# petuum/poseidon

Measured on AMD Instinct MI355X. Metric: images/sec (whole node), higher is better.
Workload: dtype bf16; 1 GPU; model=alexnet, global_batch=256, input=3x227x227, parallelism=dp1, sfb=False, hipgraph=True

## Files before the change

### poseidon_amd/ops/csrc/bindings.cpp

```cpp

#include <torch/extension.h>
#include <c10/hip/HIPStream.h>
#include <hip/hip_runtime.h>

#include <algorithm>
#include <atomic>
#include <cmath>
#include <cstdlib>
#include <utility>

#include "ps_api.h"
#include "ps_mt.h"

namespace {

using at::Tensor;

hipStream_t stream() { return c10::hip::getCurrentHIPStream().stream(); }

bool is_bf16(const Tensor& t) { return t.scalar_type() == at::kBFloat16; }

struct P {
  void* p;
  explicit P(const Tensor& t) : p(t.data_ptr()) {}
// ... 33 lines not shown
  return t_cl.permute({0, 2, 3, 1}).reshape({NP, t_cl.size(1)});
}

Tensor as_rows(const Tensor& t, int64_t* rows, int* C) {
  Tensor tc = t.dim() == 4 ? cl4(t) : t.contiguous();
  *C = (int)(t.dim() == 4 ? tc.size(1) : tc.size(-1));
  *rows = tc.numel() / *C;
  return tc;
}

Tensor weight_shadow(const Tensor& w_f32, bool bf16) {
  if (!bf16) return w_f32.contiguous();
  auto wc = w_f32.contiguous();
  Tensor out = at::empty(wc.sizes(), wc.options().dtype(at::kBFloat16));
  ps_f32_to_bf16(wc.data_ptr<float>(), out.data_ptr(), wc.numel(), stream());
  return out;
}


std::atomic<bool> g_implicit_gemm{false};
std::atomic<int64_t> g_implicit_thresh{192LL << 20};
std::atomic<int64_t> g_dgrad_fwd_thresh{128LL << 20};
std::atomic<bool> g_packed_conv{false};

void set_implicit_gemm(bool on) { g_implicit_gemm.store(on); }
void set_packed_conv(bool on) { g_packed_conv.store(on); }
void set_implicit_threshold(int64_t bytes) { g_implicit_thresh.store(bytes); }
void set_dgrad_fwd_threshold(int64_t bytes) { g_dgrad_fwd_thresh.store(bytes); }

bool deterministic() { return ps_deterministic() != 0; }
void set_deterministic(bool on) { ps_set_deterministic(on ? 1 : 0); }
int64_t float_atomic_launches(bool reset) {
  return ps_float_atomic_launches(reset ? 1 : 0);
}

void colsum_into(const Tensor& d, float* out, int64_t R, int C) {
  Tensor scratch;
  const int64_t n = ps_colsum_scratch_elems(R, C, is_bf16(d) ? 1 : 0);
  if (n > 0) scratch = at::empty({n}, d.options().dtype(at::kFloat));
  PS_CALL(colsum, is_bf16(d), P(d), out, R, C,
          n > 0 ? scratch.data_ptr<float>() : nullptr, stream());
}

const void* zero_page(const Tensor& like) {
  static Tensor z;
  if (!z.defined())
    z = at::zeros({64}, like.options().dtype(at::kByte));
// ... 139 lines not shown
    if (own) dw = t;
  }
  if (has_bias) {
    Tensor t = at::zeros({N}, x.options().dtype(at::kFloat));
    colsum_into(dyc, t.data_ptr<float>(), M, N);
    db = t;
  }
  return {dx, dw, db};
}

Tensor gemm_at_b(const Tensor& a, const Tensor& b) {
  check_float_like(a, "a");
  auto ac = a.contiguous();
  auto bc = b.contiguous();
  int M = ac.size(0), N = ac.size(1), K = bc.size(1);
  Tensor t = at::empty({N, K}, a.options().dtype(at::kFloat));
  run_gemm(ac, bc, t, nullptr, N, K, M, N, K, K, 0, 0, 0, false, false,
           1.0f, 0.0f);
  return t;
}


enum { PS_PACKED_OFF = 0, PS_PACKED_ON = 1, PS_PACKED_AUTO = -1 };

ConvPlan conv_plan_for(at::IntArrayRef x_shape, int Co, int kh, int kw,
                       int sh, int sw, int ph, int pw, int G, bool bf16,
                       int packed = PS_PACKED_AUTO) {
  TORCH_CHECK(x_shape.size() == 4 && G > 0 && x_shape[1] % G == 0 &&
              Co % G == 0, "conv channel/group mismatch");
  const ConvPolicy policy = {
      g_implicit_gemm.load(), g_implicit_thresh.load(),
      g_dgrad_fwd_thresh.load(),
      packed == PS_PACKED_AUTO ? g_packed_conv.load() : packed == PS_PACKED_ON};
  return ps_conv_plan((int)x_shape[0], (int)x_shape[1], (int)x_shape[2],
                      (int)x_shape[3], Co, kh, kw, sh, sw, ph, pw, G,
                      bf16 ? 2 : 4, policy);
}

py::dict conv_plan(std::vector<int64_t> x_shape, std::vector<int64_t> w_shape,
                   std::vector<int64_t> stride, std::vector<int64_t> pad,
                   int G, bool bf16) {
  TORCH_CHECK(w_shape.size() == 4 && stride.size() == 2 && pad.size() == 2);
  TORCH_CHECK(x_shape.size() == 4 && w_shape[1] * G == x_shape[1],
              "conv channel/group mismatch");
  const ConvPlan p = conv_plan_for(x_shape, (int)w_shape[0], (int)w_shape[2],
                                   (int)w_shape[3], (int)stride[0],
                                   (int)stride[1], (int)pad[0], (int)pad[1],
                                   G, bf16);
  py::dict d;
  d["N"] = p.g.N; d["C"] = p.g.C; d["H"] = p.g.H; d["W"] = p.g.W;
  d["Ho"] = p.g.Ho; d["Wo"] = p.g.Wo; d["G"] = p.g.G;
  d["Co"] = p.Co; d["Cg"] = p.Cg; d["Cog"] = p.Cog;
  d["Kg"] = p.Kg; d["Kcol"] = p.Kcol; d["NP"] = p.NP; d["vec"] = p.vec;
  d["is_1x1"] = p.is_1x1; d["ld_col"] = p.ld_col; d["wk_ld"] = p.wk_ld;
  d["kpad"] = p.kpad; d["implicit"] = p.implicit;
  d["Kgw_implicit"] = p.Kgw_implicit; d["dgrad_as_fwd"] = p.dgrad_as_fwd;
  d["packed"] = p.packed; d["pk_W"] = p.pk_W; d["pk_kw"] = p.pk_kw;
  d["pk_Kg"] = p.pk_Kg; d["kw_ld"] = p.kw_ld; d["c_ld"] = p.c_ld;
  d["Kgw"] = p.implicit ? p.Kgw_implicit : p.wk_ld;
  return d;
}

std::vector<int64_t> khwc_layout(int64_t Cg, int64_t kw, bool packed) {
  int kw_ld, c_ld;
  ps_khwc_layout((int)kw, (int)Cg, packed, &kw_ld, &c_ld);
  return {kw_ld, c_ld};
}

Tensor weight_khwc_tr(const Tensor& w, int G, bool bf16) {
  auto wc = w.contiguous();
  int Co = wc.size(0), Cig = wc.size(1), kh = wc.size(2), kw = wc.size(3);
  int Kg = kh * kw * Cig;
  Tensor wkT = at::empty({(int64_t)G * Kg, (int64_t)(Co / G)},
                         w.options().dtype(bf16 ? at::kBFloat16 : at::kFloat));
  PS_CALL_W(weight_to_khwc_tr, bf16, wc.data_ptr<float>(), P(wkT), Co, Cig,
          kh, kw, G, stream());
  return wkT;
}

std::vector<Tensor> conv2d_forward_ex(const Tensor& x, const Tensor& w,
                                      const c10::optional<Tensor>& bias,
// ... 11 lines not shown
  const ConvGeom& g = p.g;
  const int Co = p.Co, Cog = p.Cog;
  Tensor x_cl = (p.is_1x1 || p.implicit) ? cl4(x) : Tensor();

  const auto cdt = bf16 ? at::kBFloat16 : at::kFloat;
  Tensor wk, wkT;
  if (wk_cached.has_value() && wkT_cached.has_value() &&
      wk_cached->scalar_type() == cdt) {
    TORCH_CHECK(wk_cached->size(1) == p.wk_ld, "conv2d_forward: cached wk is ",
                wk_cached->size(1), " wide, the plan's wk_ld is ", p.wk_ld);
    wk = *wk_cached;
    wkT = *wkT_cached;
  } else {
    auto wc = w.contiguous();
    auto wkopts = w.options().dtype(cdt);
    wk = p.kpad ? at::zeros({Co, (int64_t)p.wk_ld}, wkopts)
                : at::empty({Co, (int64_t)p.wk_ld}, wkopts);
    wkT = at::empty({(int64_t)p.Kcol, (int64_t)Cog}, wkopts);
    PS_CALL_W(weight_to_khwc_both, bf16, wc.data_ptr<float>(), P(wk), P(wkT),
            Co, p.Cg, g.kh, g.kw, G, p.wk_ld, p.kw_ld, p.c_ld, stream());
  }

  Tensor colT;
  if (p.packed) {
    colT = at::empty({g.N, g.H, (int64_t)p.pk_W, PS_PK_C}, x.options());
    ps_pack_pairs_bf16(x.data_ptr(), colT.data_ptr(), g.N, g.C, g.H, g.W,
                       p.pk_W, g.pw, x.stride(0), x.stride(1), x.stride(2),
                       x.stride(3), stream());
  } else if (p.is_1x1) {
    colT = rows2d(x_cl);
  } else if (!p.implicit) {
    colT = at::empty({p.NP, (int64_t)p.ld_col}, x.options());
    const bool staged = PS_CALL(im2col_rowstage, bf16, P(x), P(colT), &g,
                                p.ld_col, x.stride(0), x.stride(1),
                                x.stride(2), x.stride(3), stream());
    if (!staged) {
      const Tensor xc = cl4(x);
      PS_CALL(im2col_nhwc, bf16, P(xc), P(colT), &g, p.ld_col, stream());
      if (p.kpad)
        PS_CALL(zero_cols, bf16, P(colT), p.NP, p.ld_col, p.Kcol, stream());
    }
  }

  Tensor y = empty_cl({g.N, Co, g.Ho, g.Wo}, x.options());
  const float* bp = nullptr;
  Tensor bc;
// ... 69 lines not shown
  for (int grp = 0; grp < G; ++grp) {
    run_gemm(dy2, wkT, dcolT, nullptr,
             (int)p.NP, Kg, Cog,
             Co, Cog, p.Kcol,
             (int64_t)grp * Cog, (int64_t)grp * Kg * Cog,
             (int64_t)grp * Kg,
             true, true, 1.0f, 0.0f);
  }
  if (!p.is_1x1)
    PS_CALL(col2im_nhwc, bf16, P(dcolT), P(dx), &g, stream());
  return dx;
}

Tensor conv2d_backward_weight_acc(const Tensor& x, const Tensor& colT,
                                  const Tensor& dy, Tensor dw_out,
                                  c10::optional<Tensor> db_out,
                                  int sh, int sw, int ph, int pw, int G,
                                  const c10::optional<Tensor>& dwk_buf,
                                  bool skip_unpack, bool skip_db) {
  check_float_like(dy, "dy");
  auto dy_cl = cl4(dy);
  const bool implicit = colT.numel() == 0 && colT.dim() == 1;
  const bool packed = colT.dim() == 4;
  const ConvPlan p = conv_plan_for(x.sizes(), (int)dw_out.size(0),
                                   (int)dw_out.size(2), (int)dw_out.size(3),
                                   sh, sw, ph, pw, G, is_bf16(dy),
                                   packed ? PS_PACKED_ON : PS_PACKED_OFF);
  TORCH_CHECK(dw_out.size(1) == p.Cg && dy_cl.size(2) == p.g.Ho &&
              dy_cl.size(3) == p.g.Wo, "conv wgrad: shape mismatch");
  const int Co = p.Co, Cog = p.Cog;
  if (packed) {
    TORCH_CHECK(p.packed && colT.is_contiguous() && is_bf16(colT) &&
                colT.size(0) == p.g.N && colT.size(1) == p.g.H &&
                colT.size(2) == p.pk_W && colT.size(3) == PS_PK_C,
                "conv wgrad: packed input does not match the plan");
  } else {
    TORCH_CHECK(implicit || colT.size(1) == p.ld_col,
                "conv wgrad: colT width does not match the plan");
  }
  const Tensor xg = packed ? colT : implicit ? cl4(x) : Tensor();
  const bool gather = implicit || packed;
  const int Kgw = implicit ? p.Kgw_implicit : p.wk_ld;

  const bool prez = dwk_buf.has_value() && dwk_buf->numel() == (int64_t)Co * Kgw;
  Tensor dwk = prez ? *dwk_buf
             : at::empty({Co, (int64_t)Kgw}, dy.options().dtype(at::kFloat));
  Tensor dy2 = rows2d(dy_cl);
  for (int grp = 0; grp < G; ++grp) {
    GatherDesc gb{};
    if (gather)
      gb = ps_gather_desc(p, PS_GATHER_WGRAD, xg.data_ptr(), zero_page(xg),
                          grp);
    run_gemm(dy2, gather ? xg : colT, dwk, nullptr,
// ... 872 lines not shown
}

PYBIND11_MODULE(TORCH_EXTENSION_NAME, m) {
  m.def("data_transform", &data_transform);
  m.def("gemm", &gemm);
  m.def("gemm_plan", &gemm_plan);
  m.def("linear_forward", &linear_forward);
  m.def("linear_backward", &linear_backward);
  m.def("gemm_at_b", &gemm_at_b);
  m.def("conv_plan", &conv_plan);
  m.def("conv2d_forward_ex", &conv2d_forward_ex);
  m.def("conv2d_backward_input", &conv2d_backward_input);
  m.def("conv2d_backward_weight_acc", &conv2d_backward_weight_acc);
  m.def("set_implicit_gemm", &set_implicit_gemm);
  m.def("set_deterministic", &set_deterministic);
  m.def("deterministic", &deterministic);
  m.def("float_atomic_launches", &float_atomic_launches);
  m.def("set_tr16_tune", &ps_gemm_set_tr_tune);
  m.def("set_implicit_threshold", &set_implicit_threshold);
  m.def("set_packed_conv", &set_packed_conv);
  m.def("khwc_layout", &khwc_layout);
  if (const char* e = std::getenv("PS_PACKED_CONV"))
    set_packed_conv(std::atoi(e) != 0);
  m.def("set_dgrad_fwd_threshold", &set_dgrad_fwd_threshold);
  m.def("concat_channels", &concat_channels);
  m.def("slice_channels", &slice_channels);
  m.def("split_channels", &split_channels);
  m.def("pool_max_forward", &pool_max_forward);
  m.def("pool_max_backward", &pool_max_backward);
  m.def("pool_ave_forward", &pool_ave_forward);
  m.def("pool_ave_backward", &pool_ave_backward);
  m.def("pool_stoch_forward_train", &pool_stoch_forward_train);
  m.def("pool_stoch_forward_test", &pool_stoch_forward_test);
  m.def("lrn_forward", &lrn_forward);
  m.def("lrn_backward", &lrn_backward);
  m.def("lrn_backward_tail", &lrn_backward_tail);
  m.def("pool_max_backward_tail", &pool_max_backward_tail);
  m.def("relu_backward_bias", &relu_backward_bias);
  m.def("set_bwd_tail_blocks", &set_bwd_tail_blocks);
  m.def("lrn_v8_ok", &ps_lrn_v8_ok);
  m.def("softmax_forward", &softmax_forward);
  m.def("softmax_backward", &softmax_backward);
  m.def("softmax_loss_forward", &softmax_loss_forward);
  m.def("softmax_loss_backward", &softmax_loss_backward);
  m.def("relu_forward", &relu_forward);
  m.def("relu_backward", &relu_backward);
// ... 31 lines not shown
```

### poseidon_amd/ops/csrc/ps_api.h

```cpp
#pragma once
#include <hip/hip_runtime.h>
#include <cstdint>

#include "ps_conv_plan.h"
#include "ps_gemm_plan.h"
#include "ps_transform.h"

struct GemmArgs {
  const void* A;
  const void* B;
  void* C;
  const float* bias;
  int M, N, K;
  int64_t lda, ldb, ldc;
  float alpha, beta;
  bool a_klast, b_klast;
  bool in_bf16;
  bool out_f32;
  const GatherDesc* gather_a;
  const GatherDesc* gather_b;
  bool relu;
  bool c_prezeroed;
};

// ... 126 lines not shown
                   hipStream_t);
void ps_nesterov_update(float*, const float*, float*, int64_t, float, float,
                        float, hipStream_t);
void ps_adagrad_update(float*, const float*, float*, int64_t, float, float,
                       float, hipStream_t);
void ps_f32_to_bf16(const float*, void*, int64_t, hipStream_t);
void ps_sgd_update_lrdev(float*, const float*, float*, int64_t, float, float,
                         float, const float*, hipStream_t);
void ps_u64_inc(void*, hipStream_t);
void ps_sgd_mt(const void* descs, const void* chunks, int nchunks, float lr,
               float mom, const float* lr_dev, hipStream_t);
void ps_zero_mt(const void* descs, const void* chunks, int nchunks,
                hipStream_t);
void ps_repack_mt(const void* descs, const void* chunks, int nchunks,
                  hipStream_t);
void ps_unpack_mt(const void* descs, const void* chunks, int nchunks,
                  hipStream_t);

void ps_data_transform_f32(const uint8_t*, const int*, const float*, float*,
                           const TransformGeom*, hipStream_t);
void ps_data_transform_bf16(const uint8_t*, const int*, const float*, void*,
                            const TransformGeom*, hipStream_t);

void ps_chan_concat4_f32(float*, void* const*, const int*, int, int, int64_t,
                         int, int, const void* const*, hipStream_t);
void ps_chan_concat4_bf16(void*, void* const*, const int*, int, int, int64_t,
                          int, int, const void* const*, hipStream_t);
void ps_chan_copy_f32(const float*, float*, int64_t, int, int, int, hipStream_t);
void ps_chan_copy_bf16(const void*, void*, int64_t, int, int, int, hipStream_t);
void ps_chan_slice_f32(const float*, float*, int64_t, int, int, int, hipStream_t);
void ps_chan_slice_bf16(const void*, void*, int64_t, int, int, int, hipStream_t);
void ps_im2col_nhwc_f32(const float*, float*, const ConvGeom*, int ldcol,
                        hipStream_t);
bool ps_im2col_rowstage_f32(const float*, float*, const ConvGeom*, int ldcol,
                            int64_t sn, int64_t sc, int64_t sh, int64_t sw,
                            hipStream_t);
bool ps_im2col_rowstage_bf16(const void*, void*, const ConvGeom*, int ldcol,
                             int64_t sn, int64_t sc, int64_t sh, int64_t sw,
                             hipStream_t);
void ps_col2im_nhwc_f32(const float*, float*, const ConvGeom*, hipStream_t);
void ps_im2col_nhwc_bf16(const void*, void*, const ConvGeom*, int ldcol,
                         hipStream_t);
void ps_col2im_nhwc_bf16(const void*, void*, const ConvGeom*, hipStream_t);
void ps_weight_to_khwc_f32(const float*, float*, int, int, int, int, hipStream_t);
void ps_weight_to_khwc_f32_bf16(const float*, void*, int, int, int, int, hipStream_t);
void ps_zero_cols_f32(float*, int64_t rows, int ld, int c_lo, hipStream_t);
// ... 23 lines not shown
```

### poseidon_amd/ops/csrc/ps_conv_plan.h

```cpp
#pragma once
#include <cstdint>

#if defined(__HIPCC__)
#define PS_HD __host__ __device__
#else
#define PS_HD
#endif

struct ConvGeom {
  int N, C, H, W;
  int Ho, Wo;
  int kh, kw, sh, sw, ph, pw;
  int G;
};

struct GatherDesc {
  const void* x;
  const void* zero;
  int C, H, W, Ho, Wo;
  int kh, kw, sh, sw, ph, pw;
  int Cg, c0;
  int kg_max;
  float inv_Cg, inv_kw, inv_Wo, inv_Ho;
};

inline void ps_fill_gather_inv(GatherDesc* g) {
  g->inv_Cg = 1.0f / g->Cg;
  g->inv_kw = 1.0f / g->kw;
  g->inv_Wo = 1.0f / g->Wo;
  g->inv_Ho = 1.0f / g->Ho;
}

struct ConvPolicy {
  bool force_implicit;
  int64_t implicit_bytes;
  int64_t dgrad_fwd_bytes;
  bool packed;
};

constexpr int PS_PK_SLOTS = 4;
constexpr int PS_PK_C = 2 * PS_PK_SLOTS;

PS_HD inline int ps_pk_chunk(int iw, int pw) { return (iw + pw) >> 1; }
PS_HD inline int ps_pk_half(int iw, int pw) { return (iw + pw) & 1; }
PS_HD inline int64_t ps_pk_x_index(int n, int ih, int iw, int c, int H,
                                   int Wp, int pw) {
  return (((int64_t)n * H + ih) * Wp + ps_pk_chunk(iw, pw)) * PS_PK_C +
         ps_pk_half(iw, pw) * PS_PK_SLOTS + c;
}
PS_HD inline int ps_khwc_col(int ky, int kx, int c, int kw_ld, int c_ld) {
  return (ky * kw_ld + kx) * c_ld + c;
}
inline void ps_khwc_layout(int kw, int Cg, bool packed, int* kw_ld,
                           int* c_ld) {
  *kw_ld = packed ? 2 * ((kw + 1) / 2) : kw;
  *c_ld = packed ? PS_PK_SLOTS : Cg;
}

struct ConvPlan {
  ConvGeom g;
  int Co, Cg, Cog;
  int Kg, Kcol;
  int64_t NP;
  int vec;
  bool is_1x1;
  int ld_col;
  int wk_ld;
  bool kpad;
  bool implicit;
  int Kgw_implicit;
  bool dgrad_as_fwd;
  bool packed;
  int pk_W;
  int pk_kw;
  int pk_Kg;
  int kw_ld, c_ld;
};

inline ConvPlan ps_conv_plan(int N, int C, int H, int W, int Co, int kh,
                             int kw, int sh, int sw, int ph, int pw, int G,
                             int elem_bytes, const ConvPolicy& policy) {
  ConvPlan p;
  p.g = {N, C, H, W, (H + 2 * ph - kh) / sh + 1, (W + 2 * pw - kw) / sw + 1,
         kh, kw, sh, sw, ph, pw, G};
  p.Co = Co;
  p.Cg = C / G;
  p.Cog = Co / G;
  p.Kg = kh * kw * p.Cg;
  p.Kcol = G * p.Kg;
  p.NP = (int64_t)N * p.g.Ho * p.g.Wo;
  p.vec = 16 / elem_bytes;
  p.is_1x1 = kh == 1 && kw == 1 && sh == 1 && sw == 1 && ph == 0 && pw == 0;
  p.ld_col = (p.is_1x1 || G != 1) ? p.Kcol : (p.Kcol + 63) & ~63;
  p.wk_ld = p.ld_col / G;
  p.kpad = p.ld_col != p.Kcol;
  const int64_t colT_bytes = p.NP * p.Kcol * elem_bytes;
  p.implicit = (policy.force_implicit || colT_bytes > policy.implicit_bytes) &&
               !p.is_1x1 && p.Cg % p.vec == 0;
  p.Kgw_implicit = (p.Kg + 63) & ~63;
  p.packed = policy.packed && G == 1 &&
             C <= PS_PK_SLOTS && elem_bytes == 2 && sw % 2 == 0 && !p.is_1x1 &&
             p.g.Ho > 0 && p.g.Wo > 0;
  p.pk_kw = (kw + 1) / 2;
  p.pk_W = (p.g.Wo - 1) * (sw / 2) + p.pk_kw;
  p.pk_Kg = kh * p.pk_kw * PS_PK_C;
  ps_khwc_layout(kw, p.Cg, p.packed, &p.kw_ld, &p.c_ld);
  if (p.packed) {
    p.implicit = false;
    p.wk_ld = (p.pk_Kg + 63) & ~63;
    p.kpad = true;
  }
  p.dgrad_as_fwd = sh == 1 && sw == 1 && !p.is_1x1 && p.Cog % p.vec == 0 &&
                   ph <= kh - 1 && pw <= kw - 1 &&
                   colT_bytes > policy.dgrad_fwd_bytes;
  return p;
}

enum ConvGatherRole {
  PS_GATHER_FWD,
  PS_GATHER_WGRAD,
  PS_GATHER_DGRAD_AS_FWD,
};

inline GatherDesc ps_gather_desc(const ConvPlan& p, ConvGatherRole role,
                                 const void* x, const void* zero, int grp) {
  const ConvGeom& g = p.g;
  GatherDesc d;
  d.x = x;
  d.zero = zero;
  d.kh = g.kh; d.kw = g.kw;
  if (role == PS_GATHER_DGRAD_AS_FWD) {
    d.C = p.Co; d.H = g.Ho; d.W = g.Wo; d.Ho = g.H; d.Wo = g.W;
    d.sh = 1; d.sw = 1; d.ph = g.kh - 1 - g.ph; d.pw = g.kw - 1 - g.pw;
    d.Cg = p.Cog; d.c0 = grp * p.Cog;
// ... 17 lines not shown
```

### poseidon_amd/ops/functional.py

```python

from __future__ import annotations

import math
import os
from typing import Optional, Tuple

import torch
import torch.nn.functional as F

_EXT = None
_EXT_ERR: Optional[str] = None


def _ext():
    global _EXT, _EXT_ERR
    if _EXT is None and _EXT_ERR is None:
        try:
            from . import _backend
            _EXT = _backend.load()
        except Exception as e:
            _EXT_ERR = str(e)
    if _EXT is None:
        raise RuntimeError(
            "poseidon_amd HIP extension is not built/loadable but a GPU op was "
            f"requested. Build it with `python setup.py build_ext --inplace` "
            f"(PYTORCH_ROCM_ARCH=gfx950). Original error: {_EXT_ERR}")
    return _EXT


def set_implicit_gemm(on: bool) -> None:
    _ext().set_implicit_gemm(bool(on))


def set_implicit_threshold(bytes_: int) -> None:
    if ext_available():
        _ext().set_implicit_threshold(int(bytes_))


_conv_policy_epoch = 0


def set_packed_conv(on: bool) -> None:
    global _conv_policy_epoch
    _ext().set_packed_conv(bool(on))
    _conv_policy_epoch += 1


def conv_policy_epoch() -> int:
    return _conv_policy_epoch


_deterministic_cpu = os.environ.get("PS_DETERMINISTIC", "0") not in ("", "0")


def set_deterministic(on: bool) -> None:
    global _deterministic_cpu, _conv_policy_epoch
    on = bool(on)
    if on == deterministic():
        return
    if ext_available():
        _ext().set_deterministic(on)
    _deterministic_cpu = on
    _conv_policy_epoch += 1
    from ..core.context import ctx
    ctx().deterministic = on


def deterministic() -> bool:
# ... 655 lines not shown
```

### setup.py

```python

import os

os.environ.setdefault("PYTORCH_ROCM_ARCH", "gfx950")

from setuptools import setup
from torch.utils.cpp_extension import BuildExtension, CUDAExtension

CSRC = os.path.join("poseidon_amd", "ops", "csrc")

sources = [
    os.path.join(CSRC, f)
    for f in [
        "bindings.cpp",
        "gemm.hip",
        "elementwise.hip",
        "pool.hip",
        "lrn.hip",
        "softmax.hip",
        "sgd.hip",
        "im2col.hip",
        "transform.hip",
    ]
]

_cxx = ["-O3"]
_ld = []
if os.environ.get("PS_SANITIZE") == "address":
    _cxx += ["-fsanitize=address", "-fno-omit-frame-pointer", "-g"]
    _ld += ["-fsanitize=address"]
elif os.environ.get("PS_SANITIZE") == "thread":
    _cxx += ["-fsanitize=thread", "-fno-omit-frame-pointer", "-g"]
    _ld += ["-fsanitize=thread"]

setup(
    name="poseidon_amd_hip",
    ext_modules=[
        CUDAExtension(
            name="poseidon_amd.ops._hip",
            sources=sources,
            extra_compile_args={
                "cxx": _cxx,
                "nvcc": ["-O3", "-std=c++17"],
            },
# ... 6 lines not shown
```

Measured before the change: 61030 images/sec.

## Add row-fused implicit bf16 conv for small-channel layers, skipping im2col

Adds a row-fused convolution path for forward and weight-gradient passes. It is used for bf16, ungrouped, non-1x1 convs whose channel count is not vector-aligned and whose im2col buffer would be large, which fits the AlexNet first layer. Instead of materialising a large im2col column matrix, each block stages a strip of input rows in LDS, double-buffered by dedicated stager waves. It gathers the GEMM operands from LDS through a k-offset table and runs MFMA directly, fusing bias and ReLU in forward. The wgrad path accumulates with float atomics, so it is not deterministic and is turned off when determinism is requested. The in-LDS gathers may limit MFMA throughput.

Measured after the change: 62240 images/sec (median of 6 runs). +2.0%, better.

```diff
diff --git a/poseidon_amd/ops/csrc/bindings.cpp b/poseidon_amd/ops/csrc/bindings.cpp
--- a/poseidon_amd/ops/csrc/bindings.cpp
+++ b/poseidon_amd/ops/csrc/bindings.cpp
@@ -79,7 +79,13 @@
 std::atomic<int64_t> g_implicit_thresh{192LL << 20};
 std::atomic<int64_t> g_dgrad_fwd_thresh{128LL << 20};
 std::atomic<bool> g_packed_conv{false};
-
+std::atomic<bool> g_rowfused_conv{true};
+std::atomic<int64_t> g_rowfused_thresh{256LL << 20};
+
+void set_rowfused_conv(bool on) { g_rowfused_conv.store(on); }
+bool rowfused_conv() { return g_rowfused_conv.load(); }
+int64_t rowfused_threshold() { return g_rowfused_thresh.load(); }
+void set_rowfused_threshold(int64_t bytes) { g_rowfused_thresh.store(bytes); }
 void set_implicit_gemm(bool on) { g_implicit_gemm.store(on); }
 void set_packed_conv(bool on) { g_packed_conv.store(on); }
 void set_implicit_threshold(int64_t bytes) { g_implicit_thresh.store(bytes); }
@@ -265,19 +271,27 @@
 
 
 enum { PS_PACKED_OFF = 0, PS_PACKED_ON = 1, PS_PACKED_AUTO = -1 };
+enum { PS_ROWFUSED_OFF = 0, PS_ROWFUSED_ON = 1, PS_ROWFUSED_AUTO = -1 };
 
 ConvPlan conv_plan_for(at::IntArrayRef x_shape, int Co, int kh, int kw,
                        int sh, int sw, int ph, int pw, int G, bool bf16,
-                       int packed = PS_PACKED_AUTO) {
+                       int packed = PS_PACKED_AUTO,
+                       int rowfused = PS_ROWFUSED_AUTO) {
   TORCH_CHECK(x_shape.size() == 4 && G > 0 && x_shape[1] % G == 0 &&
               Co % G == 0, "conv channel/group mismatch");
+  const bool rf_auto = rowfused == PS_ROWFUSED_AUTO;
   const ConvPolicy policy = {
       g_implicit_gemm.load(), g_implicit_thresh.load(),
       g_dgrad_fwd_thresh.load(),
-      packed == PS_PACKED_AUTO ? g_packed_conv.load() : packed == PS_PACKED_ON};
-  return ps_conv_plan((int)x_shape[0], (int)x_shape[1], (int)x_shape[2],
-                      (int)x_shape[3], Co, kh, kw, sh, sw, ph, pw, G,
-                      bf16 ? 2 : 4, policy);
+      packed == PS_PACKED_AUTO ? g_packed_conv.load() : packed == PS_PACKED_ON,
+      rf_auto ? g_rowfused_conv.load() : rowfused == PS_ROWFUSED_ON,
+      rf_auto ? g_rowfused_thresh.load() : 0,
+      rf_auto && ps_deterministic() != 0};
+  ConvPlan p = ps_conv_plan((int)x_shape[0], (int)x_shape[1], (int)x_shape[2],
+                            (int)x_shape[3], Co, kh, kw, sh, sw, ph, pw, G,
+                            bf16 ? 2 : 4, policy);
+  if (p.rowfused && !ps_rowfused_prepare()) p.rowfused = false;
+  return p;
 }
 
 py::dict conv_plan(std::vector<int64_t> x_shape, std::vector<int64_t> w_shape,
@@ -300,6 +314,7 @@
   d["Kgw_implicit"] = p.Kgw_implicit; d["dgrad_as_fwd"] = p.dgrad_as_fwd;
   d["packed"] = p.packed; d["pk_W"] = p.pk_W; d["pk_kw"] = p.pk_kw;
   d["pk_Kg"] = p.pk_Kg; d["kw_ld"] = p.kw_ld; d["c_ld"] = p.c_ld;
+  d["rowfused"] = p.rowfused;
   d["Kgw"] = p.implicit ? p.Kgw_implicit : p.wk_ld;
   return d;
 }
@@ -357,6 +372,27 @@
   }
 
   Tensor colT;
+  if (p.rowfused) {
+    TORCH_CHECK(x.numel() / g.N < (1LL << 31) &&
+                (g.H - 1) * x.stride(2) + (g.W - 1) * x.stride(3) +
+                (g.C - 1) * x.stride(1) < (1LL << 31),
+                "row-fused conv: one image must span < 2^31 elements");
+    TORCH_CHECK(wk.is_contiguous() && ((uintptr_t)wk.data_ptr() & 15) == 0,
+                "row-fused conv: wk must be contiguous and 16 B aligned");
+    const RowFusedTiling t = ps_rowfused_tiling(
+        g.N, g.C, g.H, g.W, Co, g.kh, g.kw, g.sh, g.sw, g.ph, g.pw, p.wk_ld);
+    Tensor y = empty_cl({g.N, Co, g.Ho, g.Wo}, x.options());
+    Tensor bc;
+    const float* bp = nullptr;
+    if (bias.has_value()) {
+      bc = bias->contiguous();
+      bp = bc.data_ptr<float>();
+    }
+    ps_conv_rowfused_fwd(&t, x.data_ptr(), x.stride(0), x.stride(1),
+                         x.stride(2), x.stride(3), wk.data_ptr(), bp,
+                         y.data_ptr(), fuse_relu ? 1 : 0, stream());
+    return {y, at::empty({0, (int64_t)p.ld_col}, x.options()), wkT};
+  }
   if (p.packed) {
     colT = at::empty({g.N, g.H, (int64_t)p.pk_W, PS_PK_C}, x.options());
     ps_pack_pairs_bf16(x.data_ptr(), colT.data_ptr(), g.N, g.C, g.H, g.W,
@@ -472,13 +508,43 @@
   auto dy_cl = cl4(dy);
   const bool implicit = colT.numel() == 0 && colT.dim() == 1;
   const bool packed = colT.dim() == 4;
+  const bool rowfused = colT.dim() == 2 && colT.size(0) == 0;
   const ConvPlan p = conv_plan_for(x.sizes(), (int)dw_out.size(0),
                                    (int)dw_out.size(2), (int)dw_out.size(3),
                                    sh, sw, ph, pw, G, is_bf16(dy),
-                                   packed ? PS_PACKED_ON : PS_PACKED_OFF);
+                                   packed ? PS_PACKED_ON : PS_PACKED_OFF,
+                                   rowfused ? PS_ROWFUSED_ON : PS_ROWFUSED_OFF);
   TORCH_CHECK(dw_out.size(1) == p.Cg && dy_cl.size(2) == p.g.Ho &&
               dy_cl.size(3) == p.g.Wo, "conv wgrad: shape mismatch");
   const int Co = p.Co, Cog = p.Cog;
+  if (rowfused) {
+    TORCH_CHECK(p.rowfused && is_bf16(x) && is_bf16(dy),
+                "conv wgrad: row-fused cache slot does not match the plan");
+    TORCH_CHECK(!ps_deterministic(),
+                "conv wgrad: the row-fused wgrad has no deterministic form");
+    const ConvGeom& g = p.g;
+    TORCH_CHECK(x.numel() / g.N < (1LL << 31) &&
+                (g.H - 1) * x.stride(2) + (g.W - 1) * x.stride(3) +
+                (g.C - 1) * x.stride(1) < (1LL << 31),
+                "row-fused conv: one image must span < 2^31 elements");
+    const int Kgw = p.wk_ld;
+    const bool prez =
+        dwk_buf.has_value() && dwk_buf->numel() == (int64_t)Co * Kgw;
+    Tensor dwk = prez ? *dwk_buf
+               : at::empty({Co, (int64_t)Kgw}, dy.options().dtype(at::kFloat));
+    const RowFusedTiling t = ps_rowfused_tiling(
+        g.N, g.C, g.H, g.W, Co, g.kh, g.kw, g.sh, g.sw, g.ph, g.pw, p.wk_ld);
+    ps_conv_rowfused_wgrad(&t, x.data_ptr(), x.stride(0), x.stride(1),
+                           x.stride(2), x.stride(3), dy_cl.data_ptr(),
+                           dwk.data_ptr<float>(), prez ? 1 : 0, stream());
+    if (!skip_unpack)
+      ps_weight_from_khwc_f32(dwk.data_ptr<float>(), dw_out.data_ptr<float>(),
+                              Co, p.Cg, g.kh, g.kw, Kgw,
+                              1.0f, p.kw_ld, p.c_ld, stream());
+    if (db_out.has_value() && !skip_db)
+      colsum_into(dy_cl, db_out->data_ptr<float>(), p.NP, Co);
+    return dwk;
+  }
   if (packed) {
     TORCH_CHECK(p.packed && colT.is_contiguous() && is_bf16(colT) &&
                 colT.size(0) == p.g.N && colT.size(1) == p.g.H &&
@@ -1397,6 +1463,13 @@
   m.def("khwc_layout", &khwc_layout);
   if (const char* e = std::getenv("PS_PACKED_CONV"))
     set_packed_conv(std::atoi(e) != 0);
+  m.def("set_rowfused_conv", &set_rowfused_conv);
+  m.def("set_rowfused_threshold", &set_rowfused_threshold);
+  m.def("rowfused_conv", &rowfused_conv);
+  m.def("rowfused_threshold", &rowfused_threshold);
+  m.def("set_rowfused_blocks", &ps_rowfused_set_blocks);
+  if (const char* e = std::getenv("PS_ROWFUSED_CONV"))
+    set_rowfused_conv(std::atoi(e) != 0);
   m.def("set_dgrad_fwd_threshold", &set_dgrad_fwd_threshold);
   m.def("concat_channels", &concat_channels);
   m.def("slice_channels", &slice_channels);
diff --git a/poseidon_amd/ops/csrc/conv_rowfused.hip b/poseidon_amd/ops/csrc/conv_rowfused.hip
--- /dev/null
+++ b/poseidon_amd/ops/csrc/conv_rowfused.hip
@@ -0,0 +1,453 @@
+
+#include "ps_common.h"
+#include "ps_api.h"
+#include "ps_rowfused.h"
+
+#include <atomic>
+#include <mutex>
+
+namespace ps {
+namespace {
+
+constexpr int RF_THREADS = PS_RF_THREADS;
+constexpr int RF_STAGERS = 256;
+
+typedef __attribute__((ext_vector_type(4))) __bf16 rf_bf16x4;
+typedef __attribute__((ext_vector_type(4))) int rf_i32x4;
+
+struct RfX {
+  const __bf16* x;
+  int64_t sn;
+  int sc, sh, sw;
+};
+
+__device__ inline __bf16 rf_read(const char* img, int pbase, int koff) {
+  return *reinterpret_cast<const __bf16*>(img + max(pbase + koff, 0));
+}
+
+typedef __bf16 rf_uvec8 __attribute__((ext_vector_type(8), aligned(2)));
+
+template <int NV, int NT>
+__device__ inline void rf_load_x(bf16x8 (&xv)[NV], const RowFusedTiling& t,
+                                 const RowFusedTile& tl, const RfX& X,
+                                 int tid, int first) {
+  const int vpr = t.rsw_ld / 8;
+  const int total = t.srows * t.C * vpr;
+  const int iw0 = tl.ow0 * t.sw - t.pw;
+  const int ih0 = tl.oh0 * t.sh - t.ph;
+  const __bf16* xn = X.x + tl.n * X.sn;
+#pragma unroll
+  for (int v = 0; v < NV; ++v) {
+    const int idx = first + tid + v * NT;
+    const int rc = idx / vpr;
+    const int sr = rc / t.C;
+    const int c = rc - sr * t.C;
+    const int ih = ih0 + sr;
+    const int iw = iw0 + (idx - rc * vpr) * 8;
+#pragma unroll
+    for (int j = 0; j < 8; ++j) xv[v][j] = (__bf16)0.0f;
+    if (idx < total && ih >= 0 && ih < t.H) {
+      const __bf16* src = xn + (ih * X.sh + c * X.sc);
+      if (X.sw == 1 && iw >= 0 && iw + 8 <= t.W) {
+        xv[v] = *reinterpret_cast<const rf_uvec8*>(src + iw);
+      } else {
+#pragma unroll
+        for (int j = 0; j < 8; ++j)
+          if (iw + j >= 0 && iw + j < t.W) xv[v][j] = src[(iw + j) * X.sw];
+      }
+    }
+  }
+}
+
+template <int NV, int NT>
+__device__ inline void rf_store_x(char* img, const bf16x8 (&xv)[NV],
+                                  const RowFusedTiling& t, int tid,
+                                  int first) {
+  const int total = t.srows * t.C * (t.rsw_ld / 8);
+#pragma unroll
+  for (int v = 0; v < NV; ++v) {
+    const int idx = first + tid + v * NT;
+    if (idx < total)
+      *reinterpret_cast<bf16x8*>(img + PS_RF_HDR + idx * 16) = xv[v];
+  }
+}
+
+constexpr int RF_FV = 6;
+__device__ inline void rf_stage_x(char* img, const RowFusedTiling& t,
+                                  const RowFusedTile& tl, const RfX& X,
+                                  int ptid) {
+  const int total = t.srows * t.C * (t.rsw_ld / 8);
+  for (int first = 0; first < total; first += RF_FV * RF_STAGERS) {
+    bf16x8 xv[RF_FV];
+    rf_load_x<RF_FV, RF_STAGERS>(xv, t, tl, X, ptid, first);
+    rf_store_x<RF_FV, RF_STAGERS>(img, xv, t, ptid, first);
+  }
+}
+
+__device__ inline void rf_zero_headers(char* xs0, int xs_bytes, int tid) {
+  if (tid < 4) reinterpret_cast<int*>(xs0)[tid] = 0;
+  else if (tid < 8) reinterpret_cast<int*>(xs0 + xs_bytes)[tid - 4] = 0;
+}
+
+template <int FN>
+__global__ __launch_bounds__(RF_THREADS)
+void conv_rowfused_fwd_k(RowFusedTiling t, RfX X,
+                         const __bf16* __restrict__ wk,
+                         const float* __restrict__ bias,
+                         __bf16* __restrict__ y, int relu, float alpha,
+                         int tpb) {
+  extern __shared__ __attribute__((aligned(16))) char smem[];
+  __bf16* wl = reinterpret_cast<__bf16*>(smem);
+  int* kofft = reinterpret_cast<int*>(smem + t.fwd_koff_off);
+  char* xs0 = smem + t.fwd_xs_off;
+  const int tid = threadIdx.x;
+  const int lane = tid & 63;
+  const int wid = __builtin_amdgcn_readfirstlane(tid >> 6);
+  const int l = lane & 15, q = lane >> 4;
+  const int64_t t0 = (int64_t)blockIdx.x * tpb;
+  const int64_t t1 = t0 + tpb < t.tiles ? t0 + tpb : t.tiles;
+  if (t0 >= t1) return;
+
+  {
+    const int vpr = t.Kpad / 8;
+    for (int i = tid; i < t.Cop * vpr; i += RF_THREADS) {
+      const int co = i / vpr;
+      const int kv = (i - co * vpr) * 8;
+      bf16x8 v;
+#pragma unroll
+      for (int j = 0; j < 8; ++j) v[j] = (__bf16)0.0f;
+      if (co < t.Co)
+        v = *reinterpret_cast<const bf16x8*>(&wk[(int64_t)co * t.Kpad + kv]);
+      *reinterpret_cast<bf16x8*>(&wl[co * t.w_ld + kv]) = v;
+    }
+    for (int k = tid; k < t.Kpad; k += RF_THREADS) kofft[k] = ps_rf_koff(t, k);
+    rf_zero_headers(xs0, t.xs_bytes, tid);
+  }
+  if (wid >= 4)
+    rf_stage_x(xs0, t, ps_rf_tile(t, t0), X, tid - RF_STAGERS);
+  int pf[2], pbf[2];
+#pragma unroll
+  for (int f = 0; f < 2; ++f) {
+    pf[f] = (wid & 3) * 32 + f * 16 + l;
+    pbf[f] = ps_rf_pbase(t, pf[f]);
+  }
+  __syncthreads();
+
+  for (int64_t ti = t0; ti < t1; ++ti) {
+    const int cur = (int)(ti - t0) & 1;
+    if (wid >= 4) {
+      if (ti + 1 < t1)
+        rf_stage_x(xs0 + (cur ^ 1) * t.xs_bytes, t, ps_rf_tile(t, ti + 1), X,
+                   tid - RF_STAGERS);
+    } else {
+      const RowFusedTile tl = ps_rf_tile(t, ti);
+      if (wid * 32 < tl.nlive) {
+        const char* img = xs0 + cur * t.xs_bytes;
+        int pb[2];
+#pragma unroll
+        for (int f = 0; f < 2; ++f)
+          pb[f] = pf[f] < tl.nlive ? pbf[f] : PS_RF_NEG;
+        f32x4 acc[2][FN] = {};
+#pragma unroll 2
+        for (int ks = 0; ks < t.Kpad; ks += 32) {
+          const rf_i32x4 k0 =
+              *reinterpret_cast<const rf_i32x4*>(&kofft[ks + q * 8]);
+          const rf_i32x4 k1 =
+              *reinterpret_cast<const rf_i32x4*>(&kofft[ks + q * 8 + 4]);
+          bf16x8 bfr[FN];
+#pragma unroll
+          for (int fn = 0; fn < FN; ++fn)
+            bfr[fn] = *reinterpret_cast<const bf16x8*>(
+                &wl[(fn * 16 + l) * t.w_ld + ks + q * 8]);
+          bf16x8 af[2];
+#pragma unroll
+          for (int f = 0; f < 2; ++f) {
+#pragma unroll
+            for (int e = 0; e < 4; ++e) {
+              af[f][e] = rf_read(img, pb[f], k0[e]);
+              af[f][4 + e] = rf_read(img, pb[f], k1[e]);
+            }
+          }
+#pragma unroll
+          for (int f = 0; f < 2; ++f)
+#pragma unroll
+            for (int fn = 0; fn < FN; ++fn)
+              acc[f][fn] = __builtin_amdgcn_mfma_f32_16x16x32_bf16(
+                  af[f], bfr[fn], acc[f][fn], 0, 0, 0);
+        }
+#pragma unroll
+        for (int f = 0; f < 2; ++f) {
+#pragma unroll
+          for (int fn = 0; fn < FN; ++fn) {
+            const int col = fn * 16 + l;
+            if (col >= t.Co) continue;
+            const float bv = bias ? bias[col] : 0.0f;
+#pragma unroll
+            for (int r = 0; r < 4; ++r) {
+              const int p = wid * 32 + f * 16 + q * 4 + r;
+              if (p >= tl.nlive) continue;
+              float v = alpha * acc[f][fn][r] + bv;
+              if (relu && v < 0.0f) v = 0.0f;
+              from_f32(v, y[(tl.pos0 + p) * t.Co + col]);
+            }
+          }
+        }
+      }
+    }
+    __syncthreads();
+  }
+}
+
+__device__ inline bf16x8 rf_tr_frag(unsigned base, int kk, int cb, int l,
+                                    int ld) {
+  const unsigned a1 =
+      base + (unsigned)(((kk + (l >> 2)) * ld + cb + 4 * (l & 3)) * 2);
+  const unsigned a2 = a1 + (unsigned)(4 * ld * 2);
+  rf_bf16x4 v1, v2;
+  asm volatile("ds_read_b64_tr_b16 %0, %2\n\t"
+               "ds_read_b64_tr_b16 %1, %3"
+               : "=&v"(v1), "=&v"(v2) : "v"(a1), "v"(a2));
+  bf16x8 f;
+#pragma unroll
+  for (int i = 0; i < 4; ++i) { f[i] = v1[i]; f[4 + i] = v2[i]; }
+  return f;
+}
+
+template <int N>
+__device__ inline void rf_tr_wait(bf16x8 (&a)[N]) {
+  asm volatile("s_waitcnt lgkmcnt(0)" ::: "memory");
+#pragma unroll
+  for (int i = 0; i < N; ++i) asm volatile("" : "+v"(a[i]));
+}
+
+template <int FN, int KF>
+__global__ __launch_bounds__(RF_THREADS)
+void conv_rowfused_wgrad_k(RowFusedTiling t, RfX X,
+                           const __bf16* __restrict__ dy,
+                           float* __restrict__ dwk, int tpb) {
+  extern __shared__ __attribute__((aligned(16))) char smem[];
+  int* ptab = reinterpret_cast<int*>(smem);
+  __bf16* dyl0 = reinterpret_cast<__bf16*>(smem + t.wg_dy_off);
+  char* xs0 = smem + t.wg_xs_off;
+  const int dy_tile = PS_RF_TM * t.dy_ld;
+  const int tid = threadIdx.x;
+  const int lane = tid & 63;
+  const int wid = __builtin_amdgcn_readfirstlane(tid >> 6);
+  const int l = lane & 15, q = lane >> 4;
+  const int64_t t0 = (int64_t)blockIdx.x * tpb;
+  const int64_t t1 = t0 + tpb < t.tiles ? t0 + tpb : t.tiles;
+  if (t0 >= t1) return;
+  rf_zero_headers(xs0, t.xs_bytes, tid);
+
+  const int my_pb = tid < PS_RF_TM ? ps_rf_pbase(t, tid) : 0;
+  const int cv8 = t.Cop / 8;
+  bf16x8 xv[PS_RF_XV], dv[PS_RF_DV];
+  auto load = [&](int64_t ti) {
+    const RowFusedTile tl = ps_rf_tile(t, ti);
+    rf_load_x<PS_RF_XV, RF_THREADS>(xv, t, tl, X, tid, 0);
+#pragma unroll
+    for (int v = 0; v < PS_RF_DV; ++v) {
+      const int idx = tid + v * RF_THREADS;
+      const int p = idx / cv8;
+      const int cv = (idx - p * cv8) * 8;
+#pragma unroll
+      for (int j = 0; j < 8; ++j) dv[v][j] = (__bf16)0.0f;
+      if (p < tl.nlive && cv < t.Co)
+        dv[v] = *reinterpret_cast<const bf16x8*>(
+            &dy[(tl.pos0 + p) * t.Co + cv]);
+    }
+  };
+  auto store = [&](int buf, int64_t ti) {
+    const RowFusedTile tl = ps_rf_tile(t, ti);
+    rf_store_x<PS_RF_XV, RF_THREADS>(xs0 + buf * t.xs_bytes, xv, t, tid,
+                                     0);
+    __bf16* dyl = dyl0 + buf * dy_tile;
+#pragma unroll
+    for (int v = 0; v < PS_RF_DV; ++v) {
+      const int idx = tid + v * RF_THREADS;
+      const int p = idx / cv8;
+      const int cv = (idx - p * cv8) * 8;
+      if (p < PS_RF_TM)
+        *reinterpret_cast<bf16x8*>(&dyl[p * t.dy_ld + cv]) = dv[v];
+    }
+    if (tid < PS_RF_TM)
+      ptab[buf * PS_RF_TM + tid] = tid < tl.nlive ? my_pb : PS_RF_NEG;
+  };
+  load(t0);
+  store(0, t0);
+
+  const int by = blockIdx.y;
+  int kofs[KF];
+  bool klive[KF];
+#pragma unroll
+  for (int i = 0; i < KF; ++i) {
+    const int kf = (by * KF + i) * 8 + wid;
+    klive[i] = kf * 16 < t.Kpad;
+    kofs[i] = klive[i] ? ps_rf_koff(t, kf * 16 + l) : PS_RF_NEG;
+  }
+  f32x4 acc[FN][KF] = {};
+  __syncthreads();
+
+  for (int64_t ti = t0; ti < t1; ++ti) {
+    const int cur = (int)(ti - t0) & 1;
+    if (ti + 1 < t1) load(ti + 1);
+    {
+      const RowFusedTile tl = ps_rf_tile(t, ti);
+      const char* img = xs0 + cur * t.xs_bytes;
+      const int* pt = ptab + cur * PS_RF_TM;
+      const unsigned dyb = (unsigned)(unsigned long long)(
+          __attribute__((address_space(3))) __bf16*)(dyl0 + cur * dy_tile);
+      for (int p0 = 0; p0 < tl.nlive; p0 += 32) {
+        const rf_i32x4 pa =
+            *reinterpret_cast<const rf_i32x4*>(&pt[p0 + q * 8]);
+        const rf_i32x4 pb =
+            *reinterpret_cast<const rf_i32x4*>(&pt[p0 + q * 8 + 4]);
+        bf16x8 af[FN];
+#pragma unroll
+        for (int fn = 0; fn < FN; ++fn)
+          af[fn] = rf_tr_frag(dyb, p0 + q * 8, fn * 16, l, t.dy_ld);
+        rf_tr_wait(af);
+#pragma unroll
+        for (int i = 0; i < KF; ++i) {
+          if (klive[i]) {
+            bf16x8 bfr;
+#pragma unroll
+            for (int e = 0; e < 4; ++e) {
+              bfr[e] = rf_read(img, pa[e], kofs[i]);
+              bfr[4 + e] = rf_read(img, pb[e], kofs[i]);
+            }
+#pragma unroll
+            for (int fn = 0; fn < FN; ++fn)
+              acc[fn][i] = __builtin_amdgcn_mfma_f32_16x16x32_bf16(
+                  af[fn], bfr, acc[fn][i], 0, 0, 0);
+          }
+        }
+      }
+    }
+    if (ti + 1 < t1) store(cur ^ 1, ti + 1);
+    __syncthreads();
+  }
+#pragma unroll
+  for (int fn = 0; fn < FN; ++fn)
+#pragma unroll
+    for (int i = 0; i < KF; ++i) {
+      if (!klive[i]) continue;
+      const int k = ((by * KF + i) * 8 + wid) * 16 + l;
+      if (k >= t.Kcol) continue;
+#pragma unroll
+      for (int r = 0; r < 4; ++r) {
+        const int co = fn * 16 + q * 4 + r;
+        if (co < t.Co)
+          atomicAdd(&dwk[(int64_t)co * t.Kpad + k], acc[fn][i][r]);
+      }
+    }
+}
+
+std::atomic<int> g_rf_blocks{0};
+
+std::atomic<int> g_rf_cus{0};
+std::once_flag g_rf_once;
+
+int rf_cu_count() {
+  const int n = g_rf_cus.load();
+  return n > 0 ? n : 256;
+}
+
+void rf_grid(const RowFusedTiling& t, int* blocks, int* tpb) {
+  const int cap = g_rf_blocks.load();
+  int64_t b = cap > 0 ? cap : rf_cu_count();
+  if (b > t.tiles) b = t.tiles;
+  *tpb = (int)((t.tiles + b - 1) / b);
+  *blocks = (int)((t.tiles + *tpb - 1) / *tpb);
+}
+
+template <typename K>
+bool rf_allow_lds(K kernel) {
+  return hipFuncSetAttribute(reinterpret_cast<const void*>(kernel),
+                             hipFuncAttributeMaxDynamicSharedMemorySize,
+                             PS_RF_LDS_MAX) == hipSuccess;
+}
+
+template <int FN>
+void rf_launch_fwd(const RowFusedTiling& t, const RfX& X, const void* wk,
+                   const float* bias, void* y, int relu, hipStream_t s) {
+  int blocks, tpb;
+  rf_grid(t, &blocks, &tpb);
+  conv_rowfused_fwd_k<FN><<<dim3((unsigned)blocks), RF_THREADS, t.fwd_lds,
+                            s>>>(t, X, (const __bf16*)wk, bias, (__bf16*)y,
+                                 relu, 1.0f, tpb);
+}
+
+template <int FN, int KF>
+void rf_launch_wgrad(const RowFusedTiling& t, const RfX& X, const void* dy,
+                     float* dwk, hipStream_t s) {
+  int blocks, tpb;
+  rf_grid(t, &blocks, &tpb);
+  const int gy = (t.Kpad / 16 + 8 * KF - 1) / (8 * KF);
+  conv_rowfused_wgrad_k<FN, KF><<<dim3((unsigned)blocks, (unsigned)gy),
+                                  RF_THREADS, t.wg_lds, s>>>(
+      t, X, (const __bf16*)dy, dwk, tpb);
+}
+
+}
+}
+
+extern "C" {
+
+void ps_rowfused_set_blocks(int n) { ps::g_rf_blocks.store(n < 0 ? 0 : n); }
+
+int ps_rowfused_prepare() {
+  using namespace ps;
+  std::call_once(g_rf_once, [] {
+    int dev = 0, n = 0;
+    if (hipGetDevice(&dev) != hipSuccess ||
+        hipDeviceGetAttribute(&n, hipDeviceAttributeMultiprocessorCount,
+                              dev) != hipSuccess || n <= 0)
+      return;
+    const bool ok =
+        rf_allow_lds(conv_rowfused_fwd_k<1>) &&
+        rf_allow_lds(conv_rowfused_fwd_k<2>) &&
+        rf_allow_lds(conv_rowfused_fwd_k<4>) &&
+        rf_allow_lds(conv_rowfused_fwd_k<6>) &&
+        rf_allow_lds(conv_rowfused_fwd_k<8>) &&
+        rf_allow_lds(conv_rowfused_wgrad_k<1, 3>) &&
+        rf_allow_lds(conv_rowfused_wgrad_k<2, 3>) &&
+        rf_allow_lds(conv_rowfused_wgrad_k<4, 3>) &&
+        rf_allow_lds(conv_rowfused_wgrad_k<6, 3>) &&
+        rf_allow_lds(conv_rowfused_wgrad_k<8, 2>);
+    if (ok) g_rf_cus.store(n);
+  });
+  return g_rf_cus.load() > 0 ? 1 : 0;
+}
+
+void ps_conv_rowfused_fwd(const RowFusedTiling* t, const void* x, int64_t sn,
+                          int64_t sc, int64_t sh, int64_t sw, const void* wk,
+                          const float* bias, void* y, int relu,
+                          hipStream_t s) {
+  const ps::RfX X = {(const __bf16*)x, sn, (int)sc, (int)sh, (int)sw};
+  const int fn = t->Cop / 16;
+  if (fn <= 1) ps::rf_launch_fwd<1>(*t, X, wk, bias, y, relu, s);
+  else if (fn <= 2) ps::rf_launch_fwd<2>(*t, X, wk, bias, y, relu, s);
+  else if (fn <= 4) ps::rf_launch_fwd<4>(*t, X, wk, bias, y, relu, s);
+  else if (fn <= 6) ps::rf_launch_fwd<6>(*t, X, wk, bias, y, relu, s);
+  else ps::rf_launch_fwd<8>(*t, X, wk, bias, y, relu, s);
+}
+
+void ps_conv_rowfused_wgrad(const RowFusedTiling* t, const void* x,
+                            int64_t sn, int64_t sc, int64_t sh, int64_t sw,
+                            const void* dy, float* dwk, int prezeroed,
+                            hipStream_t s) {
+  const ps::RfX X = {(const __bf16*)x, sn, (int)sc, (int)sh, (int)sw};
+  if (!prezeroed)
+    PS_HIP_CHECK(hipMemsetAsync(
+        dwk, 0, (size_t)t->Co * t->Kpad * sizeof(float), s));
+  ps_count_float_atomic();
+  const int fn = t->Cop / 16;
+  if (fn <= 1) ps::rf_launch_wgrad<1, 3>(*t, X, dy, dwk, s);
+  else if (fn <= 2) ps::rf_launch_wgrad<2, 3>(*t, X, dy, dwk, s);
+  else if (fn <= 4) ps::rf_launch_wgrad<4, 3>(*t, X, dy, dwk, s);
+  else if (fn <= 6) ps::rf_launch_wgrad<6, 3>(*t, X, dy, dwk, s);
+  else ps::rf_launch_wgrad<8, 2>(*t, X, dy, dwk, s);
+}
+
+}
diff --git a/poseidon_amd/ops/csrc/ps_api.h b/poseidon_amd/ops/csrc/ps_api.h
--- a/poseidon_amd/ops/csrc/ps_api.h
+++ b/poseidon_amd/ops/csrc/ps_api.h
@@ -172,6 +172,16 @@
 void ps_data_transform_bf16(const uint8_t*, const int*, const float*, void*,
                             const TransformGeom*, hipStream_t);
 
+void ps_conv_rowfused_fwd(const RowFusedTiling*, const void* x, int64_t sn,
+                          int64_t sc, int64_t sh, int64_t sw, const void* wk,
+                          const float* bias, void* y, int relu, hipStream_t);
+void ps_conv_rowfused_wgrad(const RowFusedTiling*, const void* x, int64_t sn,
+                            int64_t sc, int64_t sh, int64_t sw,
+                            const void* dy, float* dwk, int prezeroed,
+                            hipStream_t);
+int ps_rowfused_prepare();
+void ps_rowfused_set_blocks(int n);
+
 void ps_chan_concat4_f32(float*, void* const*, const int*, int, int, int64_t,
                          int, int, const void* const*, hipStream_t);
 void ps_chan_concat4_bf16(void*, void* const*, const int*, int, int, int64_t,
diff --git a/poseidon_amd/ops/csrc/ps_conv_plan.h b/poseidon_amd/ops/csrc/ps_conv_plan.h
--- a/poseidon_amd/ops/csrc/ps_conv_plan.h
+++ b/poseidon_amd/ops/csrc/ps_conv_plan.h
@@ -1,5 +1,7 @@
 #pragma once
 #include <cstdint>
+
+#include "ps_rowfused.h"
 
 #if defined(__HIPCC__)
 #define PS_HD __host__ __device__
@@ -36,6 +38,9 @@
   int64_t implicit_bytes;
   int64_t dgrad_fwd_bytes;
   bool packed;
+  bool rowfused;
+  int64_t rowfused_bytes;
+  bool deterministic;
 };
 
 constexpr int PS_PK_SLOTS = 4;
@@ -75,6 +80,7 @@
   int pk_kw;
   int pk_Kg;
   int kw_ld, c_ld;
+  bool rowfused;
 };
 
 inline ConvPlan ps_conv_plan(int N, int C, int H, int W, int Co, int kh,
@@ -110,6 +116,12 @@
     p.wk_ld = (p.pk_Kg + 63) & ~63;
     p.kpad = true;
   }
+  p.rowfused = policy.rowfused && !policy.deterministic && elem_bytes == 2 &&
+               G == 1 && C % p.vec != 0 && !p.is_1x1 && !p.packed &&
+               !p.implicit && p.g.Ho > 0 && p.g.Wo > 0 &&
+               p.NP * p.ld_col * elem_bytes >= policy.rowfused_bytes &&
+               ps_rowfused_tiling(N, C, H, W, Co, kh, kw, sh, sw, ph, pw,
+                                  p.wk_ld).ok;
   p.dgrad_as_fwd = sh == 1 && sw == 1 && !p.is_1x1 && p.Cog % p.vec == 0 &&
                    ph <= kh - 1 && pw <= kw - 1 &&
                    colT_bytes > policy.dgrad_fwd_bytes;
diff --git a/poseidon_amd/ops/csrc/ps_rowfused.h b/poseidon_amd/ops/csrc/ps_rowfused.h
--- /dev/null
+++ b/poseidon_amd/ops/csrc/ps_rowfused.h
@@ -0,0 +1,128 @@
+#pragma once
+#include <cstdint>
+
+constexpr int PS_RF_TM = 128;
+constexpr int PS_RF_THREADS = 512;
+constexpr int PS_RF_XV = 3;
+constexpr int PS_RF_DV = 4;
+constexpr int PS_RF_MAX_CO = 128;
+constexpr int PS_RF_LDS_MAX = 160 << 10;
+constexpr int PS_RF_HDR = 16;
+constexpr int PS_RF_WPAD = 8;
+constexpr int PS_RF_DYPAD = 8;
+constexpr int PS_RF_NEG = -(1 << 24);
+
+struct RowFusedTiling {
+  int C, H, W, Ho, Wo, kh, kw, sh, sw, ph, pw;
+  int Co, Cop;
+  int Kcol, Kpad;
+  int RUN;
+  int R, WS, segs;
+  int row_tiles;
+  int tiles_per_img;
+  int64_t tiles;
+  int srows;
+  int rsw;
+  int rsw_ld;
+  int xs_bytes;
+  int w_ld, dy_ld;
+  int fwd_koff_off, fwd_xs_off, fwd_lds;
+  int wg_dy_off, wg_xs_off, wg_lds;
+  bool ok;
+};
+
+struct RowFusedTile {
+  int n, oh0, ow0;
+  int nlive;
+  int64_t pos0;
+};
+
+inline int ps_rf_round_up(int v, int m) { return (v + m - 1) / m * m; }
+inline int ps_rf_co_pad(int Co) {
+  return Co <= 16 ? 16 : Co <= 32 ? 32 : Co <= 64 ? 64 : Co <= 96 ? 96 : 128;
+}
+
+inline RowFusedTiling ps_rowfused_tiling(int N, int C, int H, int W, int Co,
+                                         int kh, int kw, int sh, int sw,
+                                         int ph, int pw, int Kpad) {
+  RowFusedTiling t{};
+  t.C = C; t.H = H; t.W = W; t.kh = kh; t.kw = kw; t.sh = sh; t.sw = sw;
+  t.ph = ph; t.pw = pw;
+  t.Ho = (H + 2 * ph - kh) / sh + 1;
+  t.Wo = (W + 2 * pw - kw) / sw + 1;
+  t.Co = Co;
+  t.Cop = ps_rf_co_pad(Co);
+  t.RUN = kw * C;
+  t.Kcol = kh * t.RUN;
+  t.Kpad = Kpad;
+  if (t.Ho <= 0 || t.Wo <= 0 || Co <= 0 || Co > PS_RF_MAX_CO || Co % 8 ||
+      Kpad % 64 || Kpad < t.Kcol || N <= 0)
+    return t;
+  if (t.Wo <= PS_RF_TM) {
+    t.R = PS_RF_TM / t.Wo < t.Ho ? PS_RF_TM / t.Wo : t.Ho;
+    t.WS = t.Wo;
+    t.segs = 1;
+  } else {
+    t.R = 1;
+    t.WS = PS_RF_TM;
+    t.segs = (t.Wo + PS_RF_TM - 1) / PS_RF_TM;
+  }
+  t.row_tiles = (t.Ho + t.R - 1) / t.R;
+  t.tiles_per_img = t.row_tiles * t.segs;
+  t.tiles = (int64_t)N * t.tiles_per_img;
+  t.srows = (t.R - 1) * sh + kh;
+  t.rsw = (t.WS - 1) * sw + kw;
+  t.rsw_ld = ps_rf_round_up(t.rsw, 8);
+  const int64_t xs = PS_RF_HDR + (int64_t)t.srows * C * t.rsw_ld * 2;
+  t.w_ld = Kpad + PS_RF_WPAD;
+  t.dy_ld = t.Cop + PS_RF_DYPAD;
+  const int64_t wbytes = (int64_t)t.Cop * t.w_ld * 2;
+  const int64_t fwd = wbytes + (int64_t)Kpad * 4 + 2 * xs;
+  const int64_t dyb = (int64_t)PS_RF_TM * t.dy_ld * 2;
+  const int64_t wg = 2 * (int64_t)PS_RF_TM * 4 + 2 * dyb + 2 * xs;
+  if (fwd > PS_RF_LDS_MAX || wg > PS_RF_LDS_MAX) return t;
+  if ((int64_t)t.srows * C * (t.rsw_ld / 8) > PS_RF_THREADS * PS_RF_XV)
+    return t;
+  t.xs_bytes = (int)xs;
+  t.fwd_koff_off = (int)wbytes;
+  t.fwd_xs_off = (int)(wbytes + Kpad * 4);
+  t.fwd_lds = (int)fwd;
+  t.wg_dy_off = 2 * PS_RF_TM * 4;
+  t.wg_xs_off = (int)(t.wg_dy_off + 2 * dyb);
+  t.wg_lds = (int)wg;
+  t.ok = true;
+  return t;
+}
+
+#if defined(__HIPCC__)
+#define PS_RF_HD __host__ __device__
+#else
+#define PS_RF_HD
+#endif
+
+PS_RF_HD inline RowFusedTile ps_rf_tile(const RowFusedTiling& t, int64_t ti) {
+  RowFusedTile r;
+  r.n = (int)(ti / t.tiles_per_img);
+  const int rem = (int)(ti - (int64_t)r.n * t.tiles_per_img);
+  const int strip = rem / t.segs;
+  r.oh0 = strip * t.R;
+  r.ow0 = (rem - strip * t.segs) * t.WS;
+  const int rows = t.Ho - r.oh0 < t.R ? t.Ho - r.oh0 : t.R;
+  const int cols = t.Wo - r.ow0 < t.WS ? t.Wo - r.ow0 : t.WS;
+  r.nlive = t.segs == 1 ? rows * t.WS : cols;
+  r.pos0 = ((int64_t)r.n * t.Ho + r.oh0) * t.Wo + r.ow0;
+  return r;
+}
+
+PS_RF_HD inline int ps_rf_pbase(const RowFusedTiling& t, int p) {
+  return PS_RF_HDR +
+         ((p / t.WS) * t.sh * t.C * t.rsw_ld + (p % t.WS) * t.sw) * 2;
+}
+PS_RF_HD inline int ps_rf_koff(const RowFusedTiling& t, int k) {
+  if (k >= t.Kcol) return PS_RF_NEG;
+  return (((k / t.RUN) * t.C + k % t.C) * t.rsw_ld + (k % t.RUN) / t.C) * 2;
+}
+PS_RF_HD inline int ps_rf_addr(int pbase, int koff) {
+  const int a = pbase + koff;
+  return a < 0 ? 0 : a;
+}
diff --git a/poseidon_amd/ops/functional.py b/poseidon_amd/ops/functional.py
--- a/poseidon_amd/ops/functional.py
+++ b/poseidon_amd/ops/functional.py
@@ -44,6 +44,33 @@
     global _conv_policy_epoch
     _ext().set_packed_conv(bool(on))
     _conv_policy_epoch += 1
+
+
+ROWFUSED_THRESHOLD_DEFAULT = 256 << 20
+
+
+def set_rowfused_conv(on: bool) -> None:
+    if ext_available():
+        _ext().set_rowfused_conv(bool(on))
+
+
+def rowfused_conv() -> bool:
+    return bool(_ext().rowfused_conv()) if ext_available() else False
+
+
+def set_rowfused_threshold(bytes_: int) -> None:
+    if ext_available():
+        _ext().set_rowfused_threshold(int(bytes_))
+
+
+def rowfused_threshold() -> int:
+    return (int(_ext().rowfused_threshold()) if ext_available()
+            else ROWFUSED_THRESHOLD_DEFAULT)
+
+
+def _set_rowfused_blocks(n: int) -> None:
+    if ext_available():
+        _ext().set_rowfused_blocks(int(n))
 
 
 def conv_policy_epoch() -> int:
diff --git a/setup.py b/setup.py
--- a/setup.py
+++ b/setup.py
@@ -19,6 +19,7 @@
         "softmax.hip",
         "sgd.hip",
         "im2col.hip",
+        "conv_rowfused.hip",
         "transform.hip",
     ]
 ]
```
